# mims-harvard/Raindrop

Hardware: NVIDIA H100
Metric: samples/sec (P19-shape synthetic) training step (higher is better)
Workload: dtype f32 (tf32 operands in the ob-prop GEMMs, 3xTF32 error-compensated encoder GEMMs)

## Files before the change

raindrop_b200/csrc/rd_attn_tc.cu:

```cuda
#include <stdlib.h>

#include "rd_kernels.cuh"
#include "rd_tc_common.cuh"

namespace rd {
using namespace tc;
namespace {

constexpr int TR = 64;
constexpr int HD_MAX = 96;
constexpr int LDP = TR + 4;
constexpr int NTHR = 128;

struct AttnTcP {
  float* ctx; float* dqkv;
  const int64_t* lengths;
  int B, H, T, hd, D, ld;
  float scale, drop_p;
  const uint64_t* rng; uint32_t site;
  DropRep rep;
  unsigned long long* dbg;
};

__device__ __forceinline__ void stamp(const AttnTcP& p, int slot) {
  if (p.dbg && threadIdx.x == 0) p.dbg[(size_t)blockIdx.x * 16 + slot] = (unsigned long long)clock64();
}
__device__ __forceinline__ float ex2_approx(float x) {
  float y;
  asm("ex2.approx.ftz.f32 %0, %1;" : "=f"(y) : "f"(x));
  return y;
}

__device__ __forceinline__ void load_slice(float* s, const float* src, long long row_stride, const AttnTcP& p) {
  const int q = ((p.hd + 7) & ~7) >> 2;
  for (int v = threadIdx.x; v < TR * q; v += NTHR) {
    const int r = v / q, c = 4 * (v - r * q);
    float4 x = make_float4(0.f, 0.f, 0.f, 0.f);
    if (r < p.T && c < p.hd) x = __ldg(reinterpret_cast<const float4*>(src + r * row_stride + c));
    *reinterpret_cast<float4*>(s + r * p.ld + c) = x;
  }
}

template <int NTMAX, bool A_T, bool B_KN>
__device__ __forceinline__ void mma_rows16(float (&acc)[NTMAX][4], const float* sa, int lda, int r0, const float* sb, int ldb,
                                           int nt, int ksteps) {
  const int g = (threadIdx.x & 31) >> 2, t = threadIdx.x & 3;
#pragma unroll 1
  for (int ks = 0; ks < ksteps; ++ks) {
    const int k0 = ks * 8;
    float x0, x1, x2, x3;
    if (A_T) {
      x0 = sa[(k0 + t) * lda + r0 + g]; x1 = sa[(k0 + t) * lda + r0 + g + 8];
      x2 = sa[(k0 + t + 4) * lda + r0 + g]; x3 = sa[(k0 + t + 4) * lda + r0 + g + 8];
    } else {
      x0 = sa[(r0 + g) * lda + k0 + t]; x1 = sa[(r0 + g + 8) * lda + k0 + t];
      x2 = sa[(r0 + g) * lda + k0 + t + 4]; x3 = sa[(r0 + g + 8) * lda + k0 + t + 4];
    }
    const uint32_t ah[4] = {tf32_hi(x0), tf32_hi(x1), tf32_hi(x2), tf32_hi(x3)};
    const uint32_t al[4] = {tf32_lo(x0), tf32_lo(x1), tf32_lo(x2), tf32_lo(x3)};
#pragma unroll
    for (int j = 0; j < NTMAX; ++j) {
      if (j < nt) {
        const int n = j * 8 + g;
        const float y0 = B_KN ? sb[(k0 + t) * ldb + n] : sb[n * ldb + k0 + t];
        const float y1 = B_KN ? sb[(k0 + t + 4) * ldb + n] : sb[n * ldb + k0 + t + 4];
        mma_tf32x3(acc[j], ah, al, tf32_hi(y0), tf32_hi(y1), tf32_lo(y0), tf32_lo(y1));
      }
    }
  }
}

template <int NTMAX>
__device__ __forceinline__ void zero(float (&acc)[NTMAX][4]) {
#pragma unroll
  for (int j = 0; j < NTMAX; ++j) acc[j][0] = acc[j][1] = acc[j][2] = acc[j][3] = 0.f;
}

__device__ __forceinline__ float keep_at(const AttnTcP& p, const RngKey& key, int b, int h, int i, int j, float ik) {
  if (p.drop_p <= 0.f) return 1.f;
  if (i >= p.T || j >= p.T) return 0.f;
  return dropout_scale(key, p.site, ((uint64_t)(b * p.H + h) * p.T + i) * p.T + j, p.drop_p, ik);
}

__device__ __forceinline__ void store_rows(const float (&acc)[HD_MAX / 8][4], float* dst, long long row_stride, int r0,
                                           const AttnTcP& p) {
  const int g = (threadIdx.x & 31) >> 2, t = threadIdx.x & 3;
#pragma unroll
  for (int j = 0; j < HD_MAX / 8; ++j) {
    const int d = j * 8 + 2 * t;
#pragma unroll
    for (int i = 0; i < 2; ++i) {
      const int r = r0 + g + 8 * i;
      if (r < p.T && d < p.hd)
        *reinterpret_cast<float2*>(dst + r * row_stride + d) = make_float2(acc[j][2 * i], acc[j][2 * i + 1]);
    }
  }
}

struct RowStat { float mxs[2], sum[2]; };
__device__ __forceinline__ RowStat row_stats(const float (&s)[TR / 8][4], int nv, float sl2) {
  const int t = threadIdx.x & 3;
  RowStat r;
#pragma unroll
  for (int i = 0; i < 2; ++i) {
    float mx = -INFINITY;
#pragma unroll
    for (int j = 0; j < TR / 8; ++j)
#pragma unroll
      for (int e = 0; e < 2; ++e) if (j * 8 + 2 * t + e < nv) mx = fmaxf(mx, s[j][2 * i + e]);
    mx = fmaxf(mx, __shfl_xor_sync(0xffffffffu, mx, 1));
    mx = fmaxf(mx, __shfl_xor_sync(0xffffffffu, mx, 2));
    r.mxs[i] = mx * sl2;
    float sum = 0.f;
#pragma unroll
    for (int j = 0; j < TR / 8; ++j)
#pragma unroll
      for (int e = 0; e < 2; ++e) if (j * 8 + 2 * t + e < nv) sum += ex2_approx(fmaf(s[j][2 * i + e], sl2, -r.mxs[i]));
    sum += __shfl_xor_sync(0xffffffffu, sum, 1);
    sum += __shfl_xor_sync(0xffffffffu, sum, 2);
    r.sum[i] = sum;
  }
  return r;
}

template <bool REP>
__global__ void __launch_bounds__(NTHR) attn_tc_fwd_kernel(const float* __restrict__ qkv, const AttnTcP p) {
  extern __shared__ float sm[];
  pdl_launch_dependents();
  pdl_wait();
  stamp(p, 0);
  const int b = blockIdx.x / p.H, h = blockIdx.x - b * p.H;
  const int w = threadIdx.x >> 5, g = (threadIdx.x & 31) >> 2, t = threadIdx.x & 3;
  float* sQ = sm; float* sK = sQ + TR * p.ld; float* sV = sK + TR * p.ld; float* sP = sV + TR * p.ld;
  const long long rs = (long long)p.B * 3 * p.D;
  const float* base = qkv + (long long)b * 3 * p.D + h * p.hd;
  load_slice(sQ, base, rs, p);
  load_slice(sK, base + p.D, rs, p);
  load_slice(sV, base + 2 * p.D, rs, p);
  RngKey key = load_rng_key(p.drop_p > 0.f ? p.rng : nullptr);
  int bd = b;
  if (REP) bd = (int)(rep_remap(p.rng, p.rep, (uint32_t)b, 1, 0, &key));
  const long long len = p.lengths[b];
  const int nv = (int)(len < p.T ? (len < 0 ? 0 : len) : p.T);
  const int ksd = (p.hd + 7) >> 3;
  __syncthreads();

  float s[TR / 8][4];
  zero(s);
  mma_rows16<TR / 8, false, false>(s, sQ, p.ld, 16 * w, sK, p.ld, TR / 8, ksd);
  const float sl2 = p.scale * 1.4426950408889634f;
  const RowStat st = row_stats(s, nv, sl2);
  const float ik = p.drop_p > 0.f ? 1.f / (1.f - p.drop_p) : 1.f;
#pragma unroll
  for (int i = 0; i < 2; ++i) {
    const int r = 16 * w + g + 8 * i;
    const float invk = ((r < p.T && nv > 0) ? 1.f / st.sum[i] : 0.f);
#pragma unroll
    for (int j = 0; j < TR / 8; ++j) {
      float o[2];
#pragma unroll
      for (int e = 0; e < 2; ++e) {
        const int c = j * 8 + 2 * t + e;
        const float ex = c < nv ? ex2_approx(fmaf(s[j][2 * i + e], sl2, -st.mxs[i])) : 0.f;
        o[e] = (ex != 0.f && invk != 0.f) ? ex * invk * keep_at(p, key, bd, h, r, c, ik) : 0.f;
      }
      *reinterpret_cast<float2*>(sP + r * LDP + j * 8 + 2 * t) = make_float2(o[0], o[1]);
    }
  }
  __syncwarp();
  float o[HD_MAX / 8][4];
  zero(o);
  mma_rows16<HD_MAX / 8, false, true>(o, sP, LDP, 16 * w, sV, p.ld, ksd, TR / 8);
  store_rows(o, p.ctx + (long long)b * p.D + h * p.hd, (long long)p.B * p.D, 16 * w, p);
  stamp(p, 12);
}

__global__ void __launch_bounds__(NTHR) attn_tc_bwd_kernel(const float* __restrict__ qkv, const float* __restrict__ dctx,
                                                           const AttnTcP p) {
  extern __shared__ float sm[];
  pdl_launch_dependents();
  pdl_wait();
  stamp(p, 0);
  const int b = blockIdx.x / p.H, h = blockIdx.x - b * p.H;
  const int w = threadIdx.x >> 5, g = (threadIdx.x & 31) >> 2, t = threadIdx.x & 3;
  float* sQ = sm; float* sK = sQ + TR * p.ld; float* sV = sK + TR * p.ld; float* sG = sV + TR * p.ld;
  float* sS = sG + TR * p.ld; float* sPd = p.ld >= LDP ? sV : sS + TR * LDP;
  const long long rs = (long long)p.B * 3 * p.D;
  const float* base = qkv + (long long)b * 3 * p.D + h * p.hd;
  load_slice(sQ, base, rs, p);
  load_slice(sK, base + p.D, rs, p);
  load_slice(sV, base + 2 * p.D, rs, p);
  load_slice(sG, dctx + (long long)b * p.D + h * p.hd, (long long)p.B * p.D, p);
  const RngKey key = load_rng_key(p.drop_p > 0.f ? p.rng : nullptr);
  const long long len = p.lengths[b];
  const int nv = (int)(len < p.T ? (len < 0 ? 0 : len) : p.T);
  const int ksd = (p.hd + 7) >> 3;
  __syncthreads();

  {
    float s[TR / 8][4], dp[TR / 8][4];
    zero(s); zero(dp);
    mma_rows16<TR / 8, false, false>(s, sQ, p.ld, 16 * w, sK, p.ld, TR / 8, ksd);
    mma_rows16<TR / 8, false, false>(dp, sG, p.ld, 16 * w, sV, p.ld, TR / 8, ksd);
    __syncthreads();
    const float sl2 = p.scale * 1.4426950408889634f;
    const RowStat st = row_stats(s, nv, sl2);
    const float ik = p.drop_p > 0.f ? 1.f / (1.f - p.drop_p) : 1.f;
#pragma unroll
    for (int i = 0; i < 2; ++i) {
      const int r = 16 * w + g + 8 * i;
      const float inv = (r < p.T && nv > 0) ? 1.f / st.sum[i] : 0.f;
      float pr[TR / 8][2], m[TR / 8][2];
      float dot = 0.f;
#pragma unroll
      for (int j = 0; j < TR / 8; ++j)
#pragma unroll
        for (int e = 0; e < 2; ++e) {
          const int c = j * 8 + 2 * t + e;
          pr[j][e] = c < nv ? ex2_approx(fmaf(s[j][2 * i + e], sl2, -st.mxs[i])) * inv : 0.f;
          m[j][e] = pr[j][e] != 0.f ? keep_at(p, key, b, h, r, c, ik) : 0.f;
          dot += dp[j][2 * i + e] * m[j][e] * pr[j][e];
        }
      dot += __shfl_xor_sync(0xffffffffu, dot, 1);
      dot += __shfl_xor_sync(0xffffffffu, dot, 2);
#pragma unroll
      for (int j = 0; j < TR / 8; ++j) {
        const int c = j * 8 + 2 * t;
        *reinterpret_cast<float2*>(sPd + r * LDP + c) = make_float2(pr[j][0] * m[j][0], pr[j][1] * m[j][1]);
        *reinterpret_cast<float2*>(sS + r * LDP + c) =
            make_float2(pr[j][0] * (dp[j][2 * i] * m[j][0] - dot) * p.scale, pr[j][1] * (dp[j][2 * i + 1] * m[j][1] - dot) * p.scale);
      }
    }
  }
  __syncthreads();
  float acc[HD_MAX / 8][4];
  float* out = p.dqkv + (long long)b * 3 * p.D + h * p.hd;
  zero(acc);
  mma_rows16<HD_MAX / 8, true, true>(acc, sPd, LDP, 16 * w, sG, p.ld, ksd, TR / 8);
  store_rows(acc, out + 2 * p.D, rs, 16 * w, p);
  zero(acc);
  mma_rows16<HD_MAX / 8, false, true>(acc, sS, LDP, 16 * w, sK, p.ld, ksd, TR / 8);
  store_rows(acc, out, rs, 16 * w, p);
  zero(acc);
  mma_rows16<HD_MAX / 8, true, true>(acc, sS, LDP, 16 * w, sQ, p.ld, ksd, TR / 8);
  store_rows(acc, out + p.D, rs, 16 * w, p);
  stamp(p, 12);
}

int slice_ld(int hd) { return ((hd + 7) & ~7) + 4; }
int fwd_smem(int hd) { return (3 * TR * slice_ld(hd) + TR * LDP) * (int)sizeof(float); }
int bwd_smem(int hd) { return (4 * TR * slice_ld(hd) + (slice_ld(hd) >= LDP ? 1 : 2) * TR * LDP) * (int)sizeof(float); }

}

static unsigned long long* g_attn_dbg = nullptr;
void attn_tc_set_debug(unsigned long long* buf) { g_attn_dbg = buf; }

bool attn_tc_supported(int T, int hd) {
  static int env = -1;
  if (env < 0) { const char* e = getenv("RD_ATTN_TC"); env = (e && e[0] == '0') ? 0 : 1; }
  return env == 1 && T <= TR && hd <= HD_MAX && hd % 4 == 0 && hd >= 4;
}

int attn_tc_fwd(const float* qkv, const int64_t* lengths, int B, int H, int T, int hd, float drop_p, const uint64_t* rng,
                uint32_t site, float* ctx, cudaStream_t st, DropRep rep) {
  if (!attn_tc_supported(T, hd) || ((reinterpret_cast<uintptr_t>(qkv) | reinterpret_cast<uintptr_t>(ctx)) & 15)) {
    set_error("attn_tc_fwd: unsupported shape / alignment (T=%d hd=%d)", T, hd);
    return -2;
  }
  AttnTcP p{};
  p.ctx = ctx; p.lengths = lengths; p.B = B; p.H = H; p.T = T; p.hd = hd; p.D = H * hd; p.ld = slice_ld(hd);
  p.scale = 1.f / sqrtf((float)hd); p.drop_p = drop_p; p.rng = rng; p.site = site; p.rep = rep; p.dbg = g_attn_dbg;
  auto kern = drop_p > 0.f && rep.B ? attn_tc_fwd_kernel<true> : attn_tc_fwd_kernel<false>;
  RD_TRY(ensure_max_smem((const void*)kern, fwd_smem(HD_MAX)));
  launch_pdl(kern, dim3(B * H), dim3(NTHR), fwd_smem(hd), st, qkv, p);
  RD_CHECK_LAUNCH("attn_tc_fwd_kernel");
  return 0;
}

int attn_tc_bwd(const float* qkv, const float* dctx, const int64_t* lengths, int B, int H, int T, int hd, float drop_p,
                const uint64_t* rng, uint32_t site, float* dqkv, cudaStream_t st) {
  if (!attn_tc_supported(T, hd) ||
      ((reinterpret_cast<uintptr_t>(qkv) | reinterpret_cast<uintptr_t>(dctx) | reinterpret_cast<uintptr_t>(dqkv)) & 15)) {
    set_error("attn_tc_bwd: unsupported shape / alignment (T=%d hd=%d)", T, hd);
    return -2;
  }
  AttnTcP p{};
  p.dqkv = dqkv; p.lengths = lengths; p.B = B; p.H = H; p.T = T; p.hd = hd; p.D = H * hd; p.ld = slice_ld(hd);
  p.scale = 1.f / sqrtf((float)hd); p.drop_p = drop_p; p.rng = rng; p.site = site; p.dbg = g_attn_dbg;
  RD_TRY(ensure_max_smem((const void*)attn_tc_bwd_kernel, bwd_smem(HD_MAX)));
  launch_pdl(attn_tc_bwd_kernel, dim3(B * H), dim3(NTHR), bwd_smem(hd), st, qkv, dctx, p);
  RD_CHECK_LAUNCH("attn_tc_bwd_kernel");
  return 0;
}

}
```

Before: 169,800.

## Split attention tiles across 8 warps with column halves, cp.async staging, batched dropout bits

The tensor-core attention kernels move from 4 to 8 warps per block. Each pair of warps shares a 16-row slab and splits the key columns or head dims in half, combining row max, sum and dot through shared-memory scratch and named barriers. Q/K/V/dO slices are staged with cp.async in two commit groups, so the first GEMM can start before V and dO arrive. Dropout keep bits are precomputed once per thread from whole RNG blocks shared across lanes. This adds barrier overhead and more shared memory, and the reduction order differs from before.

```diff
diff --git a/raindrop_b200/csrc/rd_attn_tc.cu b/raindrop_b200/csrc/rd_attn_tc.cu
--- a/raindrop_b200/csrc/rd_attn_tc.cu
+++ b/raindrop_b200/csrc/rd_attn_tc.cu
@@ -10,7 +10,10 @@
 constexpr int TR = 64;
 constexpr int HD_MAX = 96;
 constexpr int LDP = TR + 4;
-constexpr int NTHR = 128;
+constexpr int NTHR = 256;
+constexpr int NS = TR / 16;
+constexpr int NTH = HD_MAX / 16;
+constexpr int XS = 12;
 
 struct AttnTcP {
   float* ctx; float* dqkv;
@@ -23,28 +26,36 @@
 };
 
 __device__ __forceinline__ void stamp(const AttnTcP& p, int slot) {
-  if (p.dbg && threadIdx.x == 0) p.dbg[(size_t)blockIdx.x * 16 + slot] = (unsigned long long)clock64();
+  if (p.dbg && threadIdx.x == 0) {
+    p.dbg[(size_t)blockIdx.x * 16 + slot] = (unsigned long long)clock64();
+    if (slot == 0 || slot == 12) {
+      unsigned long long ns;
+      asm volatile("mov.u64 %0, %%globaltimer;" : "=l"(ns));
+      p.dbg[(size_t)blockIdx.x * 16 + (slot ? 14 : 13)] = ns;
+    }
+  }
 }
 __device__ __forceinline__ float ex2_approx(float x) {
   float y;
   asm("ex2.approx.ftz.f32 %0, %1;" : "=f"(y) : "f"(x));
   return y;
 }
-
-__device__ __forceinline__ void load_slice(float* s, const float* src, long long row_stride, const AttnTcP& p) {
+__device__ __forceinline__ void pair_sync(int q) { asm volatile("bar.sync %0, 64;" ::"r"(q + 1) : "memory"); }
+
+__device__ __forceinline__ void stage_slice(float* s, const float* src, long long row_stride, const AttnTcP& p) {
   const int q = ((p.hd + 7) & ~7) >> 2;
   for (int v = threadIdx.x; v < TR * q; v += NTHR) {
     const int r = v / q, c = 4 * (v - r * q);
-    float4 x = make_float4(0.f, 0.f, 0.f, 0.f);
-    if (r < p.T && c < p.hd) x = __ldg(reinterpret_cast<const float4*>(src + r * row_stride + c));
-    *reinterpret_cast<float4*>(s + r * p.ld + c) = x;
+    if (r < p.T && c < p.hd) cp_async16(smem_u32(s + r * p.ld + c), src + r * row_stride + c, 16);
+    else *reinterpret_cast<float4*>(s + r * p.ld + c) = make_float4(0.f, 0.f, 0.f, 0.f);
   }
 }
 
 template <int NTMAX, bool A_T, bool B_KN>
 __device__ __forceinline__ void mma_rows16(float (&acc)[NTMAX][4], const float* sa, int lda, int r0, const float* sb, int ldb,
-                                           int nt, int ksteps) {
+                                           int n0, int nt, int ksteps) {
   const int g = (threadIdx.x & 31) >> 2, t = threadIdx.x & 3;
+  sb += B_KN ? 8 * n0 : 8 * n0 * ldb;
 #pragma unroll 1
   for (int ks = 0; ks < ksteps; ++ks) {
     const int k0 = ks * 8;
@@ -76,180 +87,322 @@
   for (int j = 0; j < NTMAX; ++j) acc[j][0] = acc[j][1] = acc[j][2] = acc[j][3] = 0.f;
 }
 
-__device__ __forceinline__ float keep_at(const AttnTcP& p, const RngKey& key, int b, int h, int i, int j, float ik) {
-  if (p.drop_p <= 0.f) return 1.f;
-  if (i >= p.T || j >= p.T) return 0.f;
-  return dropout_scale(key, p.site, ((uint64_t)(b * p.H + h) * p.T + i) * p.T + j, p.drop_p, ik);
-}
-
-__device__ __forceinline__ void store_rows(const float (&acc)[HD_MAX / 8][4], float* dst, long long row_stride, int r0,
-                                           const AttnTcP& p) {
+__device__ __forceinline__ uint32_t kept(uint32_t word, float p) {
+  return (float)(word >> 8) * (1.0f / 16777216.0f) >= p ? 1u : 0u;
+}
+__device__ __forceinline__ uint32_t word_of(const uint4& w, uint32_t sel) {
+  return sel == 0 ? w.x : (sel == 1 ? w.y : (sel == 2 ? w.z : w.w));
+}
+
+__device__ __forceinline__ uint32_t keep_bits(const AttnTcP& p, const RngKey& key, int bh, int r0, int j0, int nv) {
+  if (p.drop_p <= 0.f) return 0xFFFFFFFFu;
   const int g = (threadIdx.x & 31) >> 2, t = threadIdx.x & 3;
-#pragma unroll
-  for (int j = 0; j < HD_MAX / 8; ++j) {
-    const int d = j * 8 + 2 * t;
+  const uint64_t base = (uint64_t)bh * p.T;
+  uint32_t bits = 0;
+  if ((p.T & 3) == 0) {
+    const int io = t & 1, r = r0 + g + 8 * io;
+#pragma unroll
+    for (int j = 0; j < NS; ++j) {
+      const int cb = 8 * (j0 + j) + 4 * (t >> 1);
+      uint4 w = make_uint4(0u, 0u, 0u, 0u);
+      if (r < p.T && cb < nv) w = dropout_block(key, p.site, (base + r) * p.T + cb);
+      const uint32_t own0 = io ? w.z : w.x, own1 = io ? w.w : w.y;
+      const uint32_t oth0 = __shfl_xor_sync(0xffffffffu, io ? w.x : w.z, 1);
+      const uint32_t oth1 = __shfl_xor_sync(0xffffffffu, io ? w.y : w.w, 1);
+      bits |= (kept(own0, p.drop_p) | kept(own1, p.drop_p) << 1) << (16 * io + 2 * j);
+      bits |= (kept(oth0, p.drop_p) | kept(oth1, p.drop_p) << 1) << (16 * (io ^ 1) + 2 * j);
+    }
+  } else {
 #pragma unroll
     for (int i = 0; i < 2; ++i) {
       const int r = r0 + g + 8 * i;
-      if (r < p.T && d < p.hd)
+#pragma unroll
+      for (int j = 0; j < NS; ++j) {
+        const int c = 8 * (j0 + j) + 2 * t;
+        if (r < p.T && c < nv) {
+          const uint64_t idx = (base + r) * p.T + c;
+          uint4 w = dropout_block(key, p.site, idx);
+          bits |= kept(word_of(w, (uint32_t)idx & 3u), p.drop_p) << (16 * i + 2 * j);
+          if (c + 1 < nv) {
+            if (((uint32_t)idx & 3u) == 3u) w = dropout_block(key, p.site, idx + 1);
+            bits |= kept(word_of(w, (uint32_t)(idx + 1) & 3u), p.drop_p) << (16 * i + 2 * j + 1);
+          }
+        }
+      }
+    }
+  }
+  return bits;
+}
+__device__ __forceinline__ float keep_of(uint32_t bits, int i, int j, int e, float ik) {
+  return (bits >> (16 * i + 2 * j + e)) & 1u ? ik : 0.f;
+}
+
+__device__ __forceinline__ void store_rows(const float (&acc)[NTH][4], float* dst, long long row_stride, int r0, int n0,
+                                           int nt, const AttnTcP& p) {
+  const int g = (threadIdx.x & 31) >> 2, t = threadIdx.x & 3;
+#pragma unroll
+  for (int j = 0; j < NTH; ++j) {
+    const int d = (n0 + j) * 8 + 2 * t;
+#pragma unroll
+    for (int i = 0; i < 2; ++i) {
+      const int r = r0 + g + 8 * i;
+      if (j < nt && r < p.T && d < p.hd)
         *reinterpret_cast<float2*>(dst + r * row_stride + d) = make_float2(acc[j][2 * i], acc[j][2 * i + 1]);
     }
   }
 }
 
 struct RowStat { float mxs[2], sum[2]; };
-__device__ __forceinline__ RowStat row_stats(const float (&s)[TR / 8][4], int nv, float sl2) {
-  const int t = threadIdx.x & 3;
+__device__ __forceinline__ RowStat row_stats(const float (&s)[NS][4], int nv, float sl2, float* sx, int r0, int hf, int q) {
+  const int g = (threadIdx.x & 31) >> 2, t = threadIdx.x & 3, j0 = hf * NS;
   RowStat r;
 #pragma unroll
   for (int i = 0; i < 2; ++i) {
     float mx = -INFINITY;
 #pragma unroll
-    for (int j = 0; j < TR / 8; ++j)
-#pragma unroll
-      for (int e = 0; e < 2; ++e) if (j * 8 + 2 * t + e < nv) mx = fmaxf(mx, s[j][2 * i + e]);
+    for (int j = 0; j < NS; ++j)
+#pragma unroll
+      for (int e = 0; e < 2; ++e) if ((j0 + j) * 8 + 2 * t + e < nv) mx = fmaxf(mx, s[j][2 * i + e]);
     mx = fmaxf(mx, __shfl_xor_sync(0xffffffffu, mx, 1));
     mx = fmaxf(mx, __shfl_xor_sync(0xffffffffu, mx, 2));
-    r.mxs[i] = mx * sl2;
-    float sum = 0.f;
-#pragma unroll
-    for (int j = 0; j < TR / 8; ++j)
-#pragma unroll
-      for (int e = 0; e < 2; ++e) if (j * 8 + 2 * t + e < nv) sum += ex2_approx(fmaf(s[j][2 * i + e], sl2, -r.mxs[i]));
-    sum += __shfl_xor_sync(0xffffffffu, sum, 1);
-    sum += __shfl_xor_sync(0xffffffffu, sum, 2);
-    r.sum[i] = sum;
+    if (t == 0) sx[(r0 + g + 8 * i) * XS + hf] = mx;
+  }
+  pair_sync(q);
+#pragma unroll
+  for (int i = 0; i < 2; ++i) {
+    const float* x = sx + (r0 + g + 8 * i) * XS;
+    r.mxs[i] = fmaxf(x[0], x[1]) * sl2;
+  }
+  if (hf == 0) {
+#pragma unroll
+    for (int i = 0; i < 2; ++i) {
+      float sum = 0.f;
+#pragma unroll
+      for (int j = 0; j < NS; ++j)
+#pragma unroll
+        for (int e = 0; e < 2; ++e) if (j * 8 + 2 * t + e < nv) sum += ex2_approx(fmaf(s[j][2 * i + e], sl2, -r.mxs[i]));
+      sx[(r0 + g + 8 * i) * XS + 2 + t] = sum;
+    }
+  }
+  pair_sync(q);
+  if (hf == 1) {
+#pragma unroll
+    for (int i = 0; i < 2; ++i) {
+      float sum = sx[(r0 + g + 8 * i) * XS + 2 + t];
+#pragma unroll
+      for (int j = 0; j < NS; ++j)
+#pragma unroll
+        for (int e = 0; e < 2; ++e) if ((j0 + j) * 8 + 2 * t + e < nv) sum += ex2_approx(fmaf(s[j][2 * i + e], sl2, -r.mxs[i]));
+      sum += __shfl_xor_sync(0xffffffffu, sum, 1);
+      sum += __shfl_xor_sync(0xffffffffu, sum, 2);
+      if (t == 0) sx[(r0 + g + 8 * i) * XS + 6] = sum;
+      r.sum[i] = sum;
+    }
+  }
+  pair_sync(q);
+  if (hf == 0) {
+#pragma unroll
+    for (int i = 0; i < 2; ++i) r.sum[i] = sx[(r0 + g + 8 * i) * XS + 6];
   }
   return r;
 }
 
 template <bool REP>
-__global__ void __launch_bounds__(NTHR) attn_tc_fwd_kernel(const float* __restrict__ qkv, const AttnTcP p) {
+__global__ void __launch_bounds__(NTHR, 2) attn_tc_fwd_kernel(const float* __restrict__ qkv, const AttnTcP p) {
   extern __shared__ float sm[];
   pdl_launch_dependents();
   pdl_wait();
   stamp(p, 0);
   const int b = blockIdx.x / p.H, h = blockIdx.x - b * p.H;
   const int w = threadIdx.x >> 5, g = (threadIdx.x & 31) >> 2, t = threadIdx.x & 3;
+  const int q = w & 3, hf = w >> 2, r0 = 16 * q, j0 = hf * NS;
   float* sQ = sm; float* sK = sQ + TR * p.ld; float* sV = sK + TR * p.ld; float* sP = sV + TR * p.ld;
+  float* sX = sP + TR * LDP;
   const long long rs = (long long)p.B * 3 * p.D;
   const float* base = qkv + (long long)b * 3 * p.D + h * p.hd;
-  load_slice(sQ, base, rs, p);
-  load_slice(sK, base + p.D, rs, p);
-  load_slice(sV, base + 2 * p.D, rs, p);
+  stage_slice(sQ, base, rs, p);
+  stage_slice(sK, base + p.D, rs, p);
+  cp_async_commit();
+  stage_slice(sV, base + 2 * p.D, rs, p);
+  cp_async_commit();
   RngKey key = load_rng_key(p.drop_p > 0.f ? p.rng : nullptr);
   int bd = b;
   if (REP) bd = (int)(rep_remap(p.rng, p.rep, (uint32_t)b, 1, 0, &key));
   const long long len = p.lengths[b];
   const int nv = (int)(len < p.T ? (len < 0 ? 0 : len) : p.T);
   const int ksd = (p.hd + 7) >> 3;
+  const int nh0 = (ksd + 1) >> 1, n0 = hf ? nh0 : 0, nt = hf ? ksd - nh0 : nh0;
+  const uint32_t kb = keep_bits(p, key, bd * p.H + h, r0, j0, nv);
+  stamp(p, 1);
+  cp_async_wait<1>();
   __syncthreads();
-
-  float s[TR / 8][4];
+  stamp(p, 2);
+
+  float s[NS][4];
   zero(s);
-  mma_rows16<TR / 8, false, false>(s, sQ, p.ld, 16 * w, sK, p.ld, TR / 8, ksd);
+  mma_rows16<NS, false, false>(s, sQ, p.ld, r0, sK, p.ld, j0, NS, ksd);
+  stamp(p, 3);
   const float sl2 = p.scale * 1.4426950408889634f;
-  const RowStat st = row_stats(s, nv, sl2);
+  const RowStat st = row_stats(s, nv, sl2, sX, r0, hf, q);
   const float ik = p.drop_p > 0.f ? 1.f / (1.f - p.drop_p) : 1.f;
 #pragma unroll
   for (int i = 0; i < 2; ++i) {
-    const int r = 16 * w + g + 8 * i;
+    const int r = r0 + g + 8 * i;
     const float invk = ((r < p.T && nv > 0) ? 1.f / st.sum[i] : 0.f);
 #pragma unroll
-    for (int j = 0; j < TR / 8; ++j) {
+    for (int j = 0; j < NS; ++j) {
       float o[2];
 #pragma unroll
       for (int e = 0; e < 2; ++e) {
-        const int c = j * 8 + 2 * t + e;
+        const int c = (j0 + j) * 8 + 2 * t + e;
         const float ex = c < nv ? ex2_approx(fmaf(s[j][2 * i + e], sl2, -st.mxs[i])) : 0.f;
-        o[e] = (ex != 0.f && invk != 0.f) ? ex * invk * keep_at(p, key, bd, h, r, c, ik) : 0.f;
-      }
-      *reinterpret_cast<float2*>(sP + r * LDP + j * 8 + 2 * t) = make_float2(o[0], o[1]);
-    }
-  }
-  __syncwarp();
-  float o[HD_MAX / 8][4];
+        o[e] = (ex != 0.f && invk != 0.f) ? ex * invk * keep_of(kb, i, j, e, ik) : 0.f;
+      }
+      *reinterpret_cast<float2*>(sP + r * LDP + (j0 + j) * 8 + 2 * t) = make_float2(o[0], o[1]);
+    }
+  }
+  stamp(p, 4);
+  cp_async_wait<0>();
+  __syncthreads();
+  stamp(p, 5);
+  float o[NTH][4];
   zero(o);
-  mma_rows16<HD_MAX / 8, false, true>(o, sP, LDP, 16 * w, sV, p.ld, ksd, TR / 8);
-  store_rows(o, p.ctx + (long long)b * p.D + h * p.hd, (long long)p.B * p.D, 16 * w, p);
+  mma_rows16<NTH, false, true>(o, sP, LDP, r0, sV, p.ld, n0, nt, TR / 8);
+  stamp(p, 6);
+  store_rows(o, p.ctx + (long long)b * p.D + h * p.hd, (long long)p.B * p.D, r0, n0, nt, p);
   stamp(p, 12);
 }
 
-__global__ void __launch_bounds__(NTHR) attn_tc_bwd_kernel(const float* __restrict__ qkv, const float* __restrict__ dctx,
-                                                           const AttnTcP p) {
+__global__ void __launch_bounds__(NTHR, 2) attn_tc_bwd_kernel(const float* __restrict__ qkv, const float* __restrict__ dctx,
+                                                              const AttnTcP p) {
   extern __shared__ float sm[];
   pdl_launch_dependents();
   pdl_wait();
   stamp(p, 0);
   const int b = blockIdx.x / p.H, h = blockIdx.x - b * p.H;
   const int w = threadIdx.x >> 5, g = (threadIdx.x & 31) >> 2, t = threadIdx.x & 3;
+  const int q = w & 3, hf = w >> 2, r0 = 16 * q, j0 = hf * NS;
   float* sQ = sm; float* sK = sQ + TR * p.ld; float* sV = sK + TR * p.ld; float* sG = sV + TR * p.ld;
-  float* sS = sG + TR * p.ld; float* sPd = p.ld >= LDP ? sV : sS + TR * LDP;
+  float* sS = sG + TR * p.ld; float* sX = sS + TR * LDP; float* sPd = p.ld >= LDP ? sV : sX + TR * XS;
   const long long rs = (long long)p.B * 3 * p.D;
   const float* base = qkv + (long long)b * 3 * p.D + h * p.hd;
-  load_slice(sQ, base, rs, p);
-  load_slice(sK, base + p.D, rs, p);
-  load_slice(sV, base + 2 * p.D, rs, p);
-  load_slice(sG, dctx + (long long)b * p.D + h * p.hd, (long long)p.B * p.D, p);
+  stage_slice(sQ, base, rs, p);
+  stage_slice(sK, base + p.D, rs, p);
+  cp_async_commit();
+  stage_slice(sV, base + 2 * p.D, rs, p);
+  stage_slice(sG, dctx + (long long)b * p.D + h * p.hd, (long long)p.B * p.D, p);
+  cp_async_commit();
   const RngKey key = load_rng_key(p.drop_p > 0.f ? p.rng : nullptr);
   const long long len = p.lengths[b];
   const int nv = (int)(len < p.T ? (len < 0 ? 0 : len) : p.T);
   const int ksd = (p.hd + 7) >> 3;
+  const int nh0 = (ksd + 1) >> 1, n0 = hf ? nh0 : 0, nt = hf ? ksd - nh0 : nh0;
+  const uint32_t kb = keep_bits(p, key, b * p.H + h, r0, j0, nv);
+  stamp(p, 1);
+  cp_async_wait<1>();
   __syncthreads();
+  stamp(p, 2);
 
   {
-    float s[TR / 8][4], dp[TR / 8][4];
+    float s[NS][4], dp[NS][4];
     zero(s); zero(dp);
-    mma_rows16<TR / 8, false, false>(s, sQ, p.ld, 16 * w, sK, p.ld, TR / 8, ksd);
-    mma_rows16<TR / 8, false, false>(dp, sG, p.ld, 16 * w, sV, p.ld, TR / 8, ksd);
+    mma_rows16<NS, false, false>(s, sQ, p.ld, r0, sK, p.ld, j0, NS, ksd);
+    stamp(p, 3);
+    cp_async_wait<0>();
+    __syncthreads();
+    stamp(p, 4);
+    mma_rows16<NS, false, false>(dp, sG, p.ld, r0, sV, p.ld, j0, NS, ksd);
+    stamp(p, 5);
     __syncthreads();
     const float sl2 = p.scale * 1.4426950408889634f;
-    const RowStat st = row_stats(s, nv, sl2);
+    const RowStat st = row_stats(s, nv, sl2, sX, r0, hf, q);
     const float ik = p.drop_p > 0.f ? 1.f / (1.f - p.drop_p) : 1.f;
-#pragma unroll
-    for (int i = 0; i < 2; ++i) {
-      const int r = 16 * w + g + 8 * i;
+    float pr[2][NS][2], m[2][NS][2];
+#pragma unroll
+    for (int i = 0; i < 2; ++i) {
+      const int r = r0 + g + 8 * i;
       const float inv = (r < p.T && nv > 0) ? 1.f / st.sum[i] : 0.f;
-      float pr[TR / 8][2], m[TR / 8][2];
-      float dot = 0.f;
-#pragma unroll
-      for (int j = 0; j < TR / 8; ++j)
+#pragma unroll
+      for (int j = 0; j < NS; ++j)
 #pragma unroll
         for (int e = 0; e < 2; ++e) {
-          const int c = j * 8 + 2 * t + e;
-          pr[j][e] = c < nv ? ex2_approx(fmaf(s[j][2 * i + e], sl2, -st.mxs[i])) * inv : 0.f;
-          m[j][e] = pr[j][e] != 0.f ? keep_at(p, key, b, h, r, c, ik) : 0.f;
-          dot += dp[j][2 * i + e] * m[j][e] * pr[j][e];
+          const int c = (j0 + j) * 8 + 2 * t + e;
+          pr[i][j][e] = c < nv ? ex2_approx(fmaf(s[j][2 * i + e], sl2, -st.mxs[i])) * inv : 0.f;
+          m[i][j][e] = pr[i][j][e] != 0.f ? keep_of(kb, i, j, e, ik) : 0.f;
         }
-      dot += __shfl_xor_sync(0xffffffffu, dot, 1);
-      dot += __shfl_xor_sync(0xffffffffu, dot, 2);
-#pragma unroll
-      for (int j = 0; j < TR / 8; ++j) {
-        const int c = j * 8 + 2 * t;
-        *reinterpret_cast<float2*>(sPd + r * LDP + c) = make_float2(pr[j][0] * m[j][0], pr[j][1] * m[j][1]);
+    }
+    float dot[2];
+    if (hf == 0) {
+#pragma unroll
+      for (int i = 0; i < 2; ++i) {
+        float d = 0.f;
+#pragma unroll
+        for (int j = 0; j < NS; ++j)
+#pragma unroll
+          for (int e = 0; e < 2; ++e) d = __fmaf_rn(__fmul_rn(dp[j][2 * i + e], m[i][j][e]), pr[i][j][e], d);
+        sX[(r0 + g + 8 * i) * XS + 7 + t] = d;
+      }
+    }
+    pair_sync(q);
+    if (hf == 1) {
+#pragma unroll
+      for (int i = 0; i < 2; ++i) {
+        float d = sX[(r0 + g + 8 * i) * XS + 7 + t];
+#pragma unroll
+        for (int j = 0; j < NS; ++j)
+#pragma unroll
+          for (int e = 0; e < 2; ++e) d = __fmaf_rn(__fmul_rn(dp[j][2 * i + e], m[i][j][e]), pr[i][j][e], d);
+        d += __shfl_xor_sync(0xffffffffu, d, 1);
+        d += __shfl_xor_sync(0xffffffffu, d, 2);
+        if (t == 0) sX[(r0 + g + 8 * i) * XS + 11] = d;
+        dot[i] = d;
+      }
+    }
+    pair_sync(q);
+    if (hf == 0) {
+#pragma unroll
+      for (int i = 0; i < 2; ++i) dot[i] = sX[(r0 + g + 8 * i) * XS + 11];
+    }
+#pragma unroll
+    for (int i = 0; i < 2; ++i) {
+      const int r = r0 + g + 8 * i;
+#pragma unroll
+      for (int j = 0; j < NS; ++j) {
+        const int c = (j0 + j) * 8 + 2 * t;
+        float x[2];
+#pragma unroll
+        for (int e = 0; e < 2; ++e)
+          x[e] = j0 + j == TR / 8 - 1 ? __fadd_rn(__fmul_rn(dp[j][2 * i + e], m[i][j][e]), -dot[i])
+                                      : __fmaf_rn(dp[j][2 * i + e], m[i][j][e], -dot[i]);
+        *reinterpret_cast<float2*>(sPd + r * LDP + c) = make_float2(pr[i][j][0] * m[i][j][0], pr[i][j][1] * m[i][j][1]);
         *reinterpret_cast<float2*>(sS + r * LDP + c) =
-            make_float2(pr[j][0] * (dp[j][2 * i] * m[j][0] - dot) * p.scale, pr[j][1] * (dp[j][2 * i + 1] * m[j][1] - dot) * p.scale);
+            make_float2(pr[i][j][0] * x[0] * p.scale, pr[i][j][1] * x[1] * p.scale);
       }
     }
   }
   __syncthreads();
-  float acc[HD_MAX / 8][4];
+  stamp(p, 6);
+  float acc[NTH][4];
   float* out = p.dqkv + (long long)b * 3 * p.D + h * p.hd;
   zero(acc);
-  mma_rows16<HD_MAX / 8, true, true>(acc, sPd, LDP, 16 * w, sG, p.ld, ksd, TR / 8);
-  store_rows(acc, out + 2 * p.D, rs, 16 * w, p);
+  mma_rows16<NTH, true, true>(acc, sPd, LDP, r0, sG, p.ld, n0, nt, TR / 8);
+  store_rows(acc, out + 2 * p.D, rs, r0, n0, nt, p);
+  stamp(p, 7);
   zero(acc);
-  mma_rows16<HD_MAX / 8, false, true>(acc, sS, LDP, 16 * w, sK, p.ld, ksd, TR / 8);
-  store_rows(acc, out, rs, 16 * w, p);
+  mma_rows16<NTH, false, true>(acc, sS, LDP, r0, sK, p.ld, n0, nt, TR / 8);
+  store_rows(acc, out, rs, r0, n0, nt, p);
+  stamp(p, 8);
   zero(acc);
-  mma_rows16<HD_MAX / 8, true, true>(acc, sS, LDP, 16 * w, sQ, p.ld, ksd, TR / 8);
-  store_rows(acc, out + p.D, rs, 16 * w, p);
+  mma_rows16<NTH, true, true>(acc, sS, LDP, r0, sQ, p.ld, n0, nt, TR / 8);
+  store_rows(acc, out + p.D, rs, r0, n0, nt, p);
   stamp(p, 12);
 }
 
 int slice_ld(int hd) { return ((hd + 7) & ~7) + 4; }
-int fwd_smem(int hd) { return (3 * TR * slice_ld(hd) + TR * LDP) * (int)sizeof(float); }
-int bwd_smem(int hd) { return (4 * TR * slice_ld(hd) + (slice_ld(hd) >= LDP ? 1 : 2) * TR * LDP) * (int)sizeof(float); }
+int fwd_smem(int hd) { return (3 * TR * slice_ld(hd) + TR * LDP + TR * XS) * (int)sizeof(float); }
+int bwd_smem(int hd) {
+  return (4 * TR * slice_ld(hd) + (slice_ld(hd) >= LDP ? 1 : 2) * TR * LDP + TR * XS) * (int)sizeof(float);
+}
 
 }
 
```

New measurement: 183,400, median of 6. 8.0% higher.
